# nurturenature/jepsen-tigerbeetle

Hardware: AMD Instinct MI355X
Metric: histories/sec, 10k-op/64-proc cas-register histories (time-to-verdict ms in extra) (higher is better)
Workload: dtype u64

## Files before the change

jepsen-tigerbeetle_amd/csrc/open_walk_impl.h:

```cpp
#pragma once
#include "wave_env.h"
#include "tbc_internal.h"

namespace tbc {
namespace walk {

constexpr uint32_t kCandCap = 136;
constexpr uint32_t kCandWords = 8;
constexpr uint32_t kAuxWords = 80;
constexpr uint32_t kKeyWords = 32, kKeyBits = 32 * kKeyWords;
static_assert(2 * kKeyWords <= kAuxWords && kKeyWords == 32, "the map and its prefix fit the scratch; two rows of 16 lanes scan it");
constexpr uint32_t kCursorWords = 64 + 32;
WV_HD constexpr uint32_t walk_lds_words() { return kCandCap * kCandWords + kAuxWords + kCursorWords; }
static_assert(4u * walk_lds_words() * sizeof(uint32_t) <= 20u * 1024u, "eight blocks of four wavefronts a CU");
constexpr uint32_t kTogWords = 64 * 4, kRankCntWords = 24;
constexpr uint32_t kSparseCand = kCandCap - (kTogWords + kRankCntWords) / kCandWords;
constexpr int kSparseSets = 2;
static_assert(kSparseCand <= 64u * kSparseSets, "two sets of 64 candidates");
static_assert((kTogWords + kRankCntWords) % kCandWords == 0u && (kSparseCand * kCandWords) % 4u == 0u && kSparseCand >= 96u, "the toggle words of a front are 16 bytes, aligned");
#ifndef TBC_WALK_BLOCKS
#define TBC_WALK_BLOCKS 8
#endif

constexpr uint32_t kCList = 1u;
constexpr uint32_t kCTwin = 2u;
constexpr uint32_t kCRow = 4u;
constexpr uint32_t kCLook = 8u;

WV_DEV void or_slot(uint32_t& lo, uint32_t& hi, bool cond, uint32_t slot) {
  if (slot < 32u) lo = wv::opaque(lo | (cond ? (1u << slot) : 0u));
  else hi = wv::opaque(hi | (cond ? (1u << (slot - 32u)) : 0u));
}
WV_DEV uint32_t effect_key(uint32_t f, int32_t a, int32_t b) {
  return (f & 3u) | (((uint32_t)a & 0x7FFFu) << 2) | ((f == TBC_F_CAS ? ((uint32_t)b & 0x7FFFu) : 0u) << 17);
}
static_assert(kMaxRuleValue < 0x7FFF && TBC_F_READ < 3 && TBC_F_WRITE < 3 && TBC_F_CAS < 3, "effect_key packs f and two rule values into a word, and no key has all bits set");
static_assert(kLookNone <= 0xFFu, "the produced value shares a word with the flags");

WV_DEV uint32_t rank_code(uint32_t slot, uint32_t f, int32_t a, uint32_t vpad) {
  return front_rank_code(slot, f == TBC_F_READ ? (rdm_index(a, vpad) & 0xFFu) : 0xFFu);
}

template <int Q>
WV_DEV void store_entries(const wv::u32x16& r, uint64_t* row, uint32_t n) {
  WV_UNROLL
  for (int v = 0; v < 8; v++) if ((uint32_t)(8 * Q + v) < n) row[8 * Q + v] = (uint64_t)r[2 * v] | ((uint64_t)r[2 * v + 1] << 32);
}

#ifndef TBC_WALK_RUN
#define TBC_WALK_RUN 8
#endif
constexpr uint32_t kWalkRun = TBC_WALK_RUN;
static_assert(kWalkRun >= 1u, "a run has a chunk");
constexpr uint32_t kStatWalkSearch = 40, kStatWalkCarried = 41, kStatWalkCursorMiss = 42;
constexpr uint32_t kStatWalkSparse = 43, kStatWalkDense = 44, kStatWalkEmitTrips = 45, kStatWalkTwinSteps = 46, kStatWalkRounds = 47, kStatWalkTwinFind = 48;
constexpr uint32_t kStatWalkCands = 49;
constexpr uint32_t kStatWalkFindWave = 52, kStatWalkChainWave = 53;
#if defined(TBC_EMU)
#define WV_STAT_WAVE_MAX(id, n) do { for (uint32_t k_ = 1u; wv::ballot((n) >= k_) != 0ull; k_++) if (lane == 0u) wv::stat((id), 1); } while (0)
#else
#define WV_STAT_WAVE_MAX(id, n) do { (void)(n); } while (0)
#endif

WV_DEV uint32_t xor_scan(uint32_t x, uint32_t lane) {
  x ^= wv::row_shr0<1>(x); x ^= wv::row_shr0<2>(x); x ^= wv::row_shr0<4>(x); x ^= wv::row_shr0<8>(x);
  const uint32_t t0 = wv::readlane(x, 15u), t1 = wv::readlane(x, 31u), t2 = wv::readlane(x, 47u);
  return x ^ (lane >= 16u ? t0 : 0u) ^ (lane >= 32u ? t1 : 0u) ^ (lane >= 48u ? t2 : 0u);
}
#ifndef TBC_WALK_OFF_AFTER
#define TBC_WALK_OFF_AFTER 1u
#endif
#if !defined(TBC_EMU) && (defined(TBC_WALK_TWIN_LE) || defined(TBC_WALK_NO_SELF_EXCLUSION) || (TBC_WALK_OFF_AFTER != 1u))
#error "the planted mutations of the front walk are for tests/emu (TBC_EMU) only"
#endif
WV_DEV void toggle_slot(uint32_t* tog, uint32_t F_lo, uint32_t inv, uint32_t ret, uint32_t slot) {
  if (ret < F_lo) return;
  const uint32_t on = inv > F_lo ? inv - F_lo : 0u, offi = ret + TBC_WALK_OFF_AFTER - F_lo, bit = 1u << (slot & 31u), w = slot >> 5;
  wv::lds_add32(&tog[on * 4u + w], bit);
  if (ret != kInf && offi < 64u) wv::lds_add32(&tog[offi * 4u + 2u + w], bit);
}
WV_DEV void zero_toggles(uint32_t* tog, uint32_t lane) {
  const uint32_t z = wv::opaque(0u);
  *reinterpret_cast<wv::u32x4*>(tog + lane * 4u) = wv::u32x4{z, z, z, z};
}
WV_DEV uint64_t open_bits(const uint32_t* tog, uint32_t lane, bool high) {
  wv::barrier();
  const wv::u32x4 t4 = *reinterpret_cast<const wv::u32x4*>(tog + lane * 4u);
  const uint32_t lo = xor_scan(t4.x ^ t4.z, lane), hi = high ? xor_scan(t4.y ^ t4.w, lane) : 0u;
  return (uint64_t)lo | ((uint64_t)hi << 32);
}
WV_DEV uint32_t next_pending(const bool (&pend)[kSparseSets], const uint32_t (&c_fl)[kSparseSets], uint32_t NC) {
  const uint64_t b0 = wv::ballot(pend[0]), b1 = NC > 64u ? wv::ballot(pend[1]) : 0ull;
  if ((b0 | b1) == 0ull) return 0u;
  return b0 ? wv::readlane(c_fl[0], (uint32_t)__builtin_ctzll(b0)) : wv::readlane(c_fl[1], (uint32_t)__builtin_ctzll(b1));
}
WV_DEV uint32_t key_bucket(uint32_t key) { return (key * 0x9E3779B1u) >> 26; }
#if defined(TBC_EMU)
inline bool& emu_force_dense() { static bool f = false; return f; }
#endif

#if defined(TBC_EMU)
WV_DEV uint32_t opaque_uniform(uint32_t v) { return v; }
#else
WV_DEV uint32_t opaque_uniform(uint32_t v) { asm volatile("" : "+s"(v)); return v; }
#endif

#if defined(TBC_EMU)
template <class T> using ro_t = const T;
#else
template <class T> using ro_t = const __attribute__((address_space(4))) T;
#endif
template <class T>
WV_DEV ro_t<T>* read_only(const T* p) { return (ro_t<T>*)(uintptr_t)p; }

WV_DEV uint32_t first_open(const Rec* rec, uint32_t l, uint32_t hi, uint32_t ret_from) {
  while (l < hi) {
    const uint32_t mid = (l + hi) >> 1;
    if (rec[mid].ret_rank >= ret_from) hi = mid; else l = mid + 1u;
  }
  return l;
}

struct Chunk {
  ro_t<PackOpenArgs>* A;
  ro_t<Hist>* H;
  ro_t<BeamHist>* B;
  uint32_t R, F_lo, F_hi, W;
  uint32_t ret_from;
  const Rec* rec; const uint32_t* seg; const uint32_t* off;
  OpRec* lst; uint64_t* twn;
  bool want_tw;
  uint32_t V, FW;
  bool compact;
  uint64_t* rdm; uint64_t* look;
  uint32_t *cand, *aux;
  uint16_t* perm;
  uint32_t* cur_end; uint16_t* cur_left;
  uint32_t *tog, *rcnt;
};

WV_DEV uint32_t fill_candidates(const Chunk& K, uint32_t lane, bool carried) {
  const Rec* rec = K.rec;
  const uint32_t* seg = K.seg;
  const uint32_t F_lo = K.F_lo, F_hi = K.F_hi, W = K.W, V = K.V, ret_from = K.ret_from;
  const uint32_t ret_from_next = K.look ? F_lo + 64u - (kLookahead - 1u) : F_lo + 64u;
  uint32_t lo = 0, k = 0;
  if (lane == 0u) wv::stat(carried ? kStatWalkCarried : kStatWalkSearch, 1);
  if (lane < W) {
    uint32_t i;
    if (carried) { i = K.cur_end[lane]; lo = i - K.cur_left[lane]; }
    else {
      lo = first_open(rec, seg[lane] + 1u, seg[lane + 1] - 1u, ret_from);
      i = lo;
    }
#if defined(TBC_EMU)
    if (carried && lo != first_open(rec, seg[lane] + 1u, seg[lane + 1] - 1u, ret_from)) wv::stat(kStatWalkCursorMiss, 1);
    if (i > seg[lane + 1] - 1u) wv::stat(kStatWalkCursorMiss, 1);
#endif
    const uint32_t last = read_only(seg)[W] - 1u;
    for (;;) {
      const uint32_t i1 = i + 1u < last ? i + 1u : last, i2 = i + 2u < last ? i + 2u : last, i3 = i + 3u < last ? i + 3u : last;
      const uint32_t v0 = rec[i].inv_rank, v1 = rec[i1].inv_rank, v2 = rec[i2].inv_rank, v3 = rec[i3].inv_rank;
      if (v0 >= F_hi) break;
      i++;
      if (v1 >= F_hi) break;
      i++;
      if (v2 >= F_hi) break;
      i++;
      if (v3 >= F_hi) break;
      i++;
    }
    k = i - lo;
  }
  uint32_t incl = k;
  for (uint32_t d = 1; d < 64u; d <<= 1) {
    K.aux[lane] = incl;
    wv::barrier();
    const uint32_t add = lane >= d ? K.aux[lane - d] : 0u;
    wv::barrier();
    incl += add;
  }
  const uint32_t base = incl - k;
  const uint32_t NC_all = wv::readlane(incl, 63u);
  uint32_t gone = 0;
  for (uint32_t j = 0; j < k; j++) {
    const Rec r = rec[lo + j];
    gone += r.ret_rank < ret_from_next ? 1u : 0u;
    if (base + j < kCandCap) {
      const bool live = (r.cls & 2u) != 0u, isread = (r.cls & 16u) != 0u, wc = (r.cls & 8u) != 0u;
      const bool in_chunk = r.ret_rank >= F_lo;
      const bool listed = live && in_chunk && !(K.A->branch_lists && isread);
      const uint32_t vi = rdm_index(r.a, V);
      uint32_t fl = (lane << 12) | (r.prod << 24);
      if (listed) fl |= kCList;
      if (listed && wc && K.want_tw) fl |= kCTwin;
      if (live && in_chunk && isread && K.rdm && V && (vi != 0u || r.a == TBC_NIL)) fl |= kCRow | (vi << 4);
      if (K.look && (r.cls & 6u) && r.prod != kLookNone) fl |= kCLook;
      uint32_t* e = K.cand + (base + j) * kCandWords;
      e[0] = r.inv_rank; e[1] = r.ret_rank; e[2] = r.opidx; e[3] = r.f | (lane << 8);
      e[4] = (uint32_t)r.a; e[5] = (uint32_t)r.b; e[6] = fl;
      e[7] = (live && wc && in_chunk) ? effect_key(r.f, r.a, r.b) : 0xFFFFFFFFu;
    }
  }
  K.cur_end[lane] = lo + k; K.cur_left[lane] = (uint16_t)(k - gone);
  wv::barrier();
  return NC_all;
}

WV_DEV void places_by_compare(uint32_t NC, const uint32_t (&my)[3], uint32_t (&place)[3]) {
  if (NC <= 64u) {
    for (uint32_t j = 0; j < NC; j++) place[0] += wv::readlane(my[0], j) < my[0] ? 1u : 0u;
  } else if (NC <= 128u) {
    for (uint32_t j = 0; j < 64u; j++) { const uint32_t kj = wv::readlane(my[0], j); place[0] += kj < my[0] ? 1u : 0u; place[1] += kj < my[1] ? 1u : 0u; }
    for (uint32_t j = 0; j < NC - 64u; j++) { const uint32_t kj = wv::readlane(my[1], j); place[0] += kj < my[0] ? 1u : 0u; place[1] += kj < my[1] ? 1u : 0u; }
  } else {
    WV_UNROLL
    for (int s2 = 0; s2 < 3; s2++) {
      const uint32_t cnt = s2 < 2 ? 64u : NC - 128u;
      for (uint32_t j = 0; j < cnt; j++) {
        const uint32_t kj = wv::readlane(my[s2], j);
        place[0] += kj < my[0] ? 1u : 0u; place[1] += kj < my[1] ? 1u : 0u; place[2] += kj < my[2] ? 1u : 0u;
      }
    }
  }
}
WV_DEV void places_by_counting(uint32_t* aux, uint32_t NC, uint32_t lane, const uint32_t (&d)[3], uint32_t (&place)[3]) {
  if (lane < kKeyWords) aux[lane] = 0u;
  wv::barrier();
  WV_UNROLL
  for (int s = 0; s < 3; s++) if (d[s] != kInf) wv::lds_add32(&aux[d[s] >> 5], 1u << (d[s] & 31u));
  wv::barrier();
  const uint32_t wc = lane < kKeyWords ? (uint32_t)__builtin_popcount(aux[lane]) : 0u;
  uint32_t y = wc;
  y += wv::row_shr0<1>(y); y += wv::row_shr0<2>(y); y += wv::row_shr0<4>(y); y += wv::row_shr0<8>(y);
  const uint32_t row0 = wv::readlane(y, 15u);
  y += lane >= 16u ? row0 : 0u;
  const uint32_t n_live = wv::readlane(y, kKeyWords - 1u);
  if (lane < kKeyWords) aux[kKeyWords + lane] = y - wc;
  const uint64_t below = (1ull << lane) - 1ull;
  uint32_t cr_before = n_live;
  WV_UNROLL
  for (int s = 0; s < 3; s++) {
    const uint32_t idx = lane + 64u * (uint32_t)s;
    const uint64_t cr = wv::ballot(idx < NC && d[s] == kInf);
    if (d[s] == kInf) place[s] = cr_before + (uint32_t)__builtin_popcountll(cr & below);
    cr_before += (uint32_t)__builtin_popcountll(cr);
  }
  wv::barrier();
  WV_UNROLL
  for (int s = 0; s < 3; s++)
    if (d[s] != kInf) place[s] = aux[kKeyWords + (d[s] >> 5)] + (uint32_t)__builtin_popcount(aux[d[s] >> 5] & ((1u << (d[s] & 31u)) - 1u));
  wv::barrier();
}
WV_DEV void list_places(const Chunk& K, uint32_t NC, uint32_t lane, uint32_t list_order, uint32_t (&place)[3]) {
  const uint32_t wr_last = list_order == 2u ? 0x40000000u : list_order >= 16u ? 2u * (list_order - 16u) + 1u : 0u;
  const uint32_t rk_mul = list_order >= 16u ? 2u : 1u;
  const uint32_t wr_ofs = list_order == 2u ? kKeyBits / 2u : wr_last, lim_other = list_order == 2u ? kKeyBits / 2u : kKeyBits;
  uint32_t my[3];
  uint32_t d[3];
  bool outside = false;
  WV_UNROLL
  for (int s = 0; s < 3; s++) {
    const uint32_t idx = lane + 64u * (uint32_t)s;
    const uint32_t* e = K.cand + (idx < NC ? idx : 0u) * kCandWords;
    const uint32_t rt = e[1];
    const bool wr = (e[3] & 0xFFu) == TBC_F_WRITE;
    my[s] = idx >= NC ? 0xFFFFFFFFu : rt == kInf ? (0xFFFFFF00u | idx) : rt * rk_mul + (wr ? wr_last : 0u);
    const bool live = idx < NC && rt != kInf;
    const uint32_t x = rt - K.ret_from;
    const bool inside = x < kKeyBits && x * rk_mul + (wr ? wr_ofs : 0u) < (wr ? kKeyBits : lim_other);
    d[s] = (live && inside) ? x * rk_mul + (wr ? wr_ofs : 0u) : kInf;
    outside = outside || (live && !inside);
    place[s] = 0u;
  }
  if (wr_ofs < kKeyBits && wv::ballot(outside) == 0ull) places_by_counting(K.aux, NC, lane, d, place);
  else places_by_compare(NC, my, place);
  WV_UNROLL
  for (int s = 0; s < 3; s++) {
    const uint32_t idx = lane + 64u * (uint32_t)s;
    if (idx < NC) K.perm[place[s]] = (uint16_t)idx;
  }
  wv::barrier();
}

WV_DEV void sparse_flags(const Chunk& K, uint32_t NC, uint32_t lane, const uint32_t (&place)[3], uint32_t (&c_fl)[kSparseSets]) {
  WV_UNROLL
  for (int s = 0; s < kSparseSets; s++) {
    const uint32_t idx = lane + 64u * (uint32_t)s;
    if (idx < NC) c_fl[s] = K.cand[idx * kCandWords + 6u] | ((place[s] & 63u) << 18) | ((place[s] >> 6) << 9);
  }
}
WV_DEV void dense_twin_keys(const Chunk& K, uint32_t NC, uint32_t lane, uint32_t (&c_key)[3], uint32_t (&c_ret)[3]) {
  WV_UNROLL
  for (int s = 0; s < 3; s++) {
    const uint32_t idx = lane + 64u * (uint32_t)s;
    const uint32_t* e = K.cand + (idx < NC ? idx : 0u) * kCandWords;
    c_key[s] = idx < NC ? e[7] : 0xFFFFFFFFu;
    c_ret[s] = e[1];
  }
}

WV_DEV void link_twins(const Chunk& K, uint32_t NC, uint32_t lane, uint32_t (&c_key)[3], uint32_t (&c_ret)[3]) {
  uint32_t* const cand = K.cand;
  uint32_t* const tog = K.tog;
  uint32_t prev[kSparseSets] = {0xFFu, 0xFFu}, prev_ret[kSparseSets] = {0u, 0u};
  WV_UNROLL
  for (int s = 0; s < kSparseSets; s++) {
    const uint32_t idx = lane + 64u * (uint32_t)s;
    if (idx < NC) { c_key[s] = cand[idx * kCandWords + 7u]; c_ret[s] = cand[idx * kCandWords + 1u]; }
  }
  WV_UNROLL
  for (int sp = 0; sp < kSparseSets; sp++) {
    if (64u * (uint32_t)sp >= NC) continue;
    { const uint32_t z = wv::opaque(0u); tog[lane * 2u] = z; tog[lane * 2u + 1u] = z; }
    wv::barrier();
    if (c_key[sp] != 0xFFFFFFFFu) wv::lds_add32(&tog[key_bucket(c_key[sp]) * 2u + (lane >> 5)], 1u << (lane & 31u));
    wv::barrier();
    WV_UNROLL
    for (int s = 0; s < kSparseSets; s++) {
      uint64_t mk = 0ull;
      if (c_key[s] != 0xFFFFFFFFu) {
        const uint32_t hb = key_bucket(c_key[s]);
        mk = (uint64_t)tog[hb * 2u] | ((uint64_t)tog[hb * 2u + 1u] << 32);
      }
      WV_STAT_WAVE_MAX(kStatWalkFindWave, (uint32_t)__builtin_popcountll(mk));
      while (mk) {
        const uint32_t u = 64u * (uint32_t)sp + (uint32_t)__builtin_ctzll(mk);
        mk &= mk - 1ull;
        const uint32_t* eu = cand + u * kCandWords;
        const uint32_t ru = eu[1];
        wv::stat(kStatWalkTwinFind, 1);
#if defined(TBC_WALK_TWIN_LE)
        if (eu[7] == c_key[s] && ru <= c_ret[s] && (prev[s] == 0xFFu || ru > prev_ret[s])) { prev[s] = u; prev_ret[s] = ru; }
#else
        if (eu[7] == c_key[s] && ru < c_ret[s] && (prev[s] == 0xFFu || ru > prev_ret[s])) { prev[s] = u; prev_ret[s] = ru; }
#endif
      }
    }
    wv::barrier();
  }
  WV_UNROLL
  for (int s = 0; s < kSparseSets; s++) if (lane + 64u * (uint32_t)s < NC) cand[(lane + 64u * (uint32_t)s) * kCandWords + 7u] = prev[s];
  wv::barrier();
}

struct Front {
  uint32_t F, Fc; bool active;
  uint32_t pos0, px, need, xprod, di, x, xf; int32_t xa;
};
WV_DEV Front front_of(const Chunk& K, uint32_t lane) {
  const auto& A = *K.A;
  const auto* H = K.H;
  Front f;
  f.F = K.F_lo + lane;
  f.active = f.F < K.F_hi;
  f.Fc = f.active ? f.F : K.F_hi - 1u;
  f.pos0 = K.off[f.Fc];
  f.px = A.ret_slot[H->ret_off + f.Fc];
  f.need = kLookNone; f.xprod = kLookNone; f.di = 0; f.x = 0; f.xf = kFNone; f.xa = 0;
  if (K.look || K.compact) {
    f.x = A.ret_op[H->ret_off + f.Fc];
    f.xf = A.f[H->op_off + f.x];
    f.xa = A.a[H->op_off + f.x];
  }
  if (K.look) {
    const int32_t xb = A.b[H->op_off + f.x];
    const uint32_t xinv = A.scratch[H->frame_off + f.x];
    f.need = look_need(f.xf, f.xa); f.xprod = look_prod(f.xf, f.xa, xb);
    f.di = f.F - xinv < 255u ? f.F - xinv : 255u;
  }
  return f;
}
WV_DEV void store_look(const Chunk& K, const Front& f, uint64_t pm, uint32_t dmin) {
  if (f.active && K.look) {
    pm &= ~(1ull << (f.px & 63u));
    K.look[(uint64_t)f.F * 2u] = look_word0(f.px, f.need, f.xprod, f.di, dmin);
    K.look[(uint64_t)f.F * 2u + 1u] = pm;
  }
}

WV_DEV void sparse_read_rows(const Chunk& K, uint32_t NC, uint32_t lane, const Front& f, const uint32_t (&c_fl)[kSparseSets]) {
  uint64_t* const row = K.rdm ? K.rdm + (uint64_t)f.F * K.FW : nullptr;
  const uint32_t n_row = K.compact ? 6u : K.V;
  uint32_t made = 0u;
  bool pend[kSparseSets];
  WV_UNROLL
  for (int s = 0; s < kSparseSets; s++) pend[s] = (c_fl[s] & kCRow) != 0u;
  for (uint32_t fl; (fl = next_pending(pend, c_fl, NC)) != 0u;) {
    const uint32_t v = (fl >> 4) & 31u;
    if (lane == 0u) wv::stat(kStatWalkRounds, 1);
    zero_toggles(K.tog, lane);
    wv::barrier();
    WV_UNROLL
    for (int s = 0; s < kSparseSets; s++)
      if (pend[s] && ((c_fl[s] >> 4) & 31u) == v) { const uint32_t* e = K.cand + (lane + 64u * (uint32_t)s) * kCandWords; toggle_slot(K.tog, K.F_lo, e[0], e[1], (c_fl[s] >> 12) & 63u); pend[s] = false; }
    const uint64_t open = open_bits(K.tog, lane, K.W > 32u);
    if (f.active && v < n_row) row[v] = open;
    made |= 1u << v;
    wv::barrier();
  }
  if (K.rdm)
    for (uint32_t v = 0; v < n_row; v++) if (!((made >> v) & 1u) && f.active) row[v] = 0ull;
}
WV_DEV void sparse_producers(const Chunk& K, uint32_t NC, uint32_t lane, const Front& f, const uint32_t (&c_fl)[kSparseSets]) {
  static_assert(kLookahead == 8u, "a front's window of invocation ranks is eight bytes");
  uint32_t* const rcnt = K.rcnt;
  uint64_t pm = 0ull;
  uint32_t dmin = 255u;
  bool pend[kSparseSets];
  WV_UNROLL
  for (int s = 0; s < kSparseSets; s++) pend[s] = (c_fl[s] & kCLook) != 0u;
  for (uint32_t fl; (fl = next_pending(pend, c_fl, NC)) != 0u;) {
    const uint32_t v = fl >> 24;
    const bool mine = f.active && f.need == v;
    if (wv::ballot(mine) == 0ull) {
      WV_UNROLL
      for (int s = 0; s < kSparseSets; s++) if ((c_fl[s] >> 24) == v) pend[s] = false;
      continue;
    }
    if (lane == 0u) wv::stat(kStatWalkRounds, 1);
    zero_toggles(K.tog, lane);
    if (lane < kRankCntWords) rcnt[lane] = 0u;
    wv::barrier();
    WV_UNROLL
    for (int s = 0; s < kSparseSets; s++)
      if (pend[s] && (c_fl[s] >> 24) == v) {
        const uint32_t* e = K.cand + (lane + 64u * (uint32_t)s) * kCandWords;
        const uint32_t inv = e[0];
        toggle_slot(K.tog, K.F_lo, inv, e[1], (c_fl[s] >> 12) & 63u);
        if (inv + (kLookahead - 1u) >= K.F_lo) {
          const uint32_t ri = inv + (kLookahead - 1u) - K.F_lo;
          wv::lds_add32(&rcnt[ri >> 2], 1u << (8u * (ri & 3u)));
        }
        pend[s] = false;
      }
    const uint64_t open = open_bits(K.tog, lane, K.W > 32u);
    if (mine) {
      pm = open;
      const uint32_t wb = lane >> 2, sh = 8u * (lane & 3u);
      const uint64_t lo64 = (uint64_t)rcnt[wb] | ((uint64_t)rcnt[wb + 1u] << 32);
      uint64_t xb = sh ? ((lo64 >> sh) | ((uint64_t)rcnt[wb + 2u] << (64u - sh))) : lo64;
#if !defined(TBC_WALK_NO_SELF_EXCLUSION)
      if (f.xprod == f.need && f.di < kLookahead) xb -= 1ull << (8u * (kLookahead - 1u - f.di));
#endif
      dmin = xb ? (uint32_t)__builtin_clzll(xb) >> 3 : 255u;
    }
    wv::barrier();
  }
  store_look(K, f, pm, dmin);
}
WV_DEV uint32_t sparse_lists(const Chunk& K, uint32_t NC, uint32_t lane, const Front& f, const uint32_t (&c_fl)[kSparseSets], bool by_ret, uint32_t pos) {
  const uint32_t* const cand = K.cand;
  const uint32_t F = f.F;
  WV_UNROLL
  for (int g = 0; g < kSparseSets; g++) {
    if (64u * (uint32_t)g >= NC) continue;
    zero_toggles(K.tog, lane);
    wv::barrier();
    WV_UNROLL
    for (int s = 0; s < kSparseSets; s++)
      if ((c_fl[s] & kCList) && ((c_fl[s] >> 9) & 3u) == (uint32_t)g) { const uint32_t* e = cand + (lane + 64u * (uint32_t)s) * kCandWords; toggle_slot(K.tog, K.F_lo, e[0], e[1], (c_fl[s] >> 18) & 63u); }
    const uint64_t open = open_bits(K.tog, lane, true);
    uint64_t cur = f.active ? open : 0ull;
    wv::barrier();
    WV_NOUNROLL
    while (wv::ballot(cur != 0ull) != 0ull) {
      if (lane == 0u) wv::stat(kStatWalkEmitTrips, 1);
      uint32_t chain_steps = 0u;
      if (cur != 0ull) {
        const uint32_t p = 64u * (uint32_t)g + (uint32_t)__builtin_ctzll(cur);
        cur &= cur - 1ull;
        const uint32_t* e = cand + (by_ret ? (uint32_t)K.perm[p] : p) * kCandWords;
        OpRec o; o.op = e[2]; o.f_slot = e[3] | (e[1] == F ? kAtFront : 0u); o.a = (int32_t)e[4]; o.b = (int32_t)e[5];
        K.lst[pos] = o;
        if (K.twn) {
          uint64_t tw = 0ull;
          for (uint32_t u = e[7] & 0xFFu; u != 0xFFu;) {
            const uint32_t* eu = cand + u * kCandWords;
            wv::stat(kStatWalkTwinSteps, 1);
            chain_steps++;
            if (eu[1] < F) break;
            if (eu[0] <= F) tw |= 1ull << ((eu[3] >> 8) & 63u);
#if defined(TBC_WALK_TWIN_LE)
            if ((eu[7] & 0xFFu) == u) break;
#endif
            u = eu[7] & 0xFFu;
          }
          K.twn[pos] = tw;
        }
        pos++;
      }
      WV_STAT_WAVE_MAX(kStatWalkChainWave, chain_steps);
    }
  }
  return pos;
}

template <int VCAP>
WV_DEV uint32_t dense_loop(const Chunk& K, uint32_t NC, uint32_t lane, const Front& f, const uint32_t (&c_key)[3], const uint32_t (&c_ret)[3], bool by_ret, uint32_t pos) {
  const uint32_t* const cand = K.cand;
  const uint32_t F = f.F;
  const bool active = f.active;
  wv::u32x16 r0, r1, r2, r3;
  WV_UNROLL
  for (int i = 0; i < 16; i++) { r0[i] = 0u; r1[i] = 0u; r2[i] = 0u; r3[i] = 0u; }
  uint32_t pm_lo = 0u, pm_hi = 0u, dmin = 255u;
  WV_NOUNROLL
  for (uint32_t t = 0; t < NC; t++) {
    const uint32_t* e = cand + (by_ret ? (uint32_t)K.perm[t] : t) * kCandWords;
    const uint32_t inv = e[0], ret = e[1];
    const uint32_t fl = wv::readfirstlane(e[6]);
    const uint32_t slot = (fl >> 12) & 63u;
    const bool member = active && inv <= F && F <= ret;
    if (fl & kCList) {
      uint32_t tw_lo = 0u, tw_hi = 0u;
      if (fl & kCTwin) {
        const uint32_t key_t = e[7];
        uint64_t s0 = wv::ballot(c_key[0] == key_t && c_ret[0] < ret && c_ret[0] >= inv);
        uint64_t s1 = 0ull, s2 = 0ull;
        if (NC > 64u) s1 = wv::ballot(c_key[1] == key_t && c_ret[1] < ret && c_ret[1] >= inv);
        if (NC > 128u) s2 = wv::ballot(c_key[2] == key_t && c_ret[2] < ret && c_ret[2] >= inv);
        while (s0 | s1 | s2) {
          uint32_t u;
          if (s0) { u = (uint32_t)__builtin_ctzll(s0); s0 &= s0 - 1ull; }
          else if (s1) { u = 64u + (uint32_t)__builtin_ctzll(s1); s1 &= s1 - 1ull; }
          else { u = 128u + (uint32_t)__builtin_ctzll(s2); s2 &= s2 - 1ull; }
          const uint32_t* eu = cand + u * kCandWords;
          const bool mu = eu[0] <= F && F <= eu[1];
          or_slot(tw_lo, tw_hi, mu, (wv::readfirstlane(eu[6]) >> 12) & 63u);
        }
      }
      if (member) {
        OpRec o; o.op = e[2]; o.f_slot = e[3] | (ret == F ? kAtFront : 0u); o.a = (int32_t)e[4]; o.b = (int32_t)e[5];
        K.lst[pos] = o;
        if (K.twn) K.twn[pos] = (uint64_t)tw_lo | ((uint64_t)tw_hi << 32);
        pos++;
      }
    }
    if (fl & kCRow)
    {
      const uint32_t w = ((fl >> 4) & 31u) * 2u + (slot >> 5), bit = member ? (1u << (slot & 31u)) : 0u;
      if constexpr (VCAP <= 8) r0[w & 15u] |= bit;
      else {
        const uint32_t q = w >> 4;
        if (q == 0u) r0[w & 15u] |= bit; else if (q == 1u) r1[w & 15u] |= bit; else if (q == 2u) r2[w & 15u] |= bit; else r3[w & 15u] |= bit;
      }
    }
    if (fl & kCLook) {
      const bool hit = (fl >> 24) == f.need;
      or_slot(pm_lo, pm_hi, member && hit, slot);
      const uint32_t dist = F - inv;
      if (hit && dist < kLookahead && e[2] != f.x) dmin = dist < dmin ? dist : dmin;
    }
  }
  if (active && K.rdm) {
    uint64_t* row = K.rdm + (uint64_t)F * K.FW;
    const uint32_t n_row = K.compact ? 6u : K.V;
    store_entries<0>(r0, row, n_row);
    if constexpr (VCAP > 8) { store_entries<1>(r1, row, n_row); store_entries<2>(r2, row, n_row); store_entries<3>(r3, row, n_row); }
  }
  store_look(K, f, (uint64_t)pm_lo | ((uint64_t)pm_hi << 32), dmin);
  return pos;
}

WV_DEV void compact_tail(const Chunk& K, uint32_t lane, const Front& f, bool by_ret, uint32_t nl) {
  const auto& A = *K.A;
  const auto* H = K.H;
  uint32_t* const aux = K.aux;
  if (by_ret) wv::barrier();
  aux[lane] = f.active ? rank_code(f.px, f.xf, f.xa, K.V) : (7u << 6);
  if (lane < kFrontCompactRanks - 1u) {
    const uint32_t G = K.F_lo + 64u + lane;
    uint32_t code = 7u << 6;
    if (G < K.R) {
      const uint32_t gx = A.ret_op[H->ret_off + G];
      code = rank_code(A.ret_slot[H->ret_off + G], A.f[H->op_off + gx], A.a[H->op_off + gx], K.V);
    }
    aux[64u + lane] = code;
  }
  wv::barrier();
  uint64_t w7 = 0ull;
  WV_UNROLL
  for (uint32_t l = kFrontCompactRanks; l-- > 0u;) w7 |= (uint64_t)aux[lane + l] << (9u * l);
  const uint64_t w6 = front_word6(f.pos0, nl, A.ncr[K.B->off_off + f.Fc]);
  if (f.active && K.rdm) {
    uint64_t* row = K.rdm + (uint64_t)f.F * K.FW;
    row[6] = w6; row[7] = w7;
  }
}

template <int VCAP>
WV_DEV bool walk_chunk(const PackOpenArgs& A_, uint32_t h, uint32_t c, uint32_t* lds, uint32_t lane, bool carried) {
  const auto& A = *wv::cold(A_);
  const auto* H = read_only(&A.hist[h]);
  const auto* B = read_only(&A.bh[h]);
  const uint32_t R = H->n_ret;
  const uint32_t F_lo = c * 64u;
  if (H->status != 0 || B->status != 0 || F_lo >= R) return false;
  Chunk K;
  K.A = &A; K.H = H; K.B = B;
  K.R = R; K.F_lo = F_lo; K.F_hi = F_lo + 64u < R ? F_lo + 64u : R;
  K.W = H->n_slots;
  K.rec = A.rec + H->rec_off;
  K.seg = A.seg + H->seg_off;
  K.off = A.off + B->off_off;
  K.lst = A.lst + B->lst_off;
  K.twn = A.twn ? A.twn + B->lst_off : nullptr;
  K.want_tw = K.twn != nullptr;
  K.V = A.vpad;
  K.FW = A.front_words ? A.front_words : K.V;
  K.compact = A.front_compact != 0u;
  K.rdm = (A.rdm && (K.V || K.compact)) ? A.rdm + H->op_off * K.FW : nullptr;
  K.look = A.look ? A.look + look_off(H->op_off, h, 1u) : nullptr;
  K.ret_from = K.look ? (F_lo >= kLookahead - 1u ? F_lo - (kLookahead - 1u) : 0u) : F_lo;
  K.cand = lds;
  K.aux = lds + kCandCap * kCandWords;
  K.perm = reinterpret_cast<uint16_t*>(K.aux);
  K.cur_end = K.aux + kAuxWords;
  K.cur_left = reinterpret_cast<uint16_t*>(K.cur_end + 64);
  K.tog = K.cand + kSparseCand * kCandWords;
  K.rcnt = K.tog + kTogWords;

  const uint32_t NC_all = fill_candidates(K, lane, carried);
  const uint32_t NC = NC_all < kCandCap ? NC_all : kCandCap;
  const uint32_t list_order = A.order_of ? A.order_of[h] : A.list_order;
  const bool by_ret = list_order != 0u;
  uint32_t place[3] = {lane, lane + 64u, lane + 128u};
  if (by_ret) list_places(K, NC, lane, list_order, place);

  bool sparse = VCAP <= 8 && NC_all <= kSparseCand;
#if defined(TBC_EMU)
  if (emu_force_dense()) sparse = false;
#endif
  uint32_t c_fl[kSparseSets] = {0u, 0u};
  uint32_t c_key[3] = {0xFFFFFFFFu, 0xFFFFFFFFu, 0xFFFFFFFFu}, c_ret[3] = {0u, 0u, 0u};
  if (sparse) sparse_flags(K, NC, lane, place, c_fl);
  else if (K.want_tw) dense_twin_keys(K, NC, lane, c_key, c_ret);
  if constexpr (VCAP <= 8) if (sparse && K.want_tw) link_twins(K, NC, lane, c_key, c_ret);
  if (lane == 0u) wv::stat(sparse ? kStatWalkSparse : kStatWalkDense, 1);
  if (lane == 0u) wv::stat(kStatWalkCands + (NC_all > 64u ? 1u : 0u) + (NC_all > kSparseCand ? 1u : 0u), 1);

  const Front f = front_of(K, lane);
  uint32_t pos = f.pos0;
  bool dense = true;
  if constexpr (VCAP <= 8) if (sparse) {
    dense = false;
    sparse_read_rows(K, NC, lane, f, c_fl);
    sparse_producers(K, NC, lane, f, c_fl);
    pos = sparse_lists(K, NC, lane, f, c_fl, by_ret, pos);
  }
  if (dense) pos = dense_loop<VCAP>(K, NC, lane, f, c_key, c_ret, by_ret, pos);
  if (K.compact) compact_tail(K, lane, f, by_ret, pos - f.pos0);
  return F_lo + 64u < R;
}

template <int VCAP>
WV_DEV void walk_wave(const PackOpenArgs& A, uint32_t wid, uint32_t* lds, uint32_t lane) {
  const uint32_t cph = A.chunks_per_hist;
  const uint32_t hr = wid / cph, c = wid - hr * cph, h = A.h0 + hr;
  if (h >= A.n_hist) return;
  (void)walk_chunk<VCAP>(A, h, c, lds, lane, false);
}

WV_HD constexpr uint32_t walk_runs_per_hist(uint32_t chunks_per_hist, uint32_t run = kWalkRun) { return (chunks_per_hist + run - 1u) / run; }

template <int VCAP, uint32_t RUN = kWalkRun>
WV_DEV void walk_run(const PackOpenArgs& A, uint32_t run_id, uint32_t* lds, uint32_t lane) {
  const uint32_t rph = walk_runs_per_hist(A.chunks_per_hist, RUN);
  const uint32_t hr = run_id / rph, c0 = (run_id - hr * rph) * RUN, h = A.h0 + hr;
  if (h >= A.n_hist) return;
  WV_NOUNROLL
  for (uint32_t j = 0; j < RUN; j++) {
    if (!walk_chunk<VCAP>(A, opaque_uniform(h), c0 + j, lds, wv::opaque(lane), j != 0u)) break;
    wv::barrier();
  }
}

}
}
```

Before: 410,200.

## Redistribute sparse list emission across lanes by global entry rank

The sparse emission loop no longer has each lane (front) walk its own open candidates serially. It computes a wave-wide prefix sum of per-front counts, then assigns every output entry to a lane in batches of 64. Each lane finds its front through an LDS mark array and a max-scan, then locates the k-th set bit of that front's open mask. The aim is to remove divergence where one busy front serialises the wave, and to make the lst/twn writes contiguous across lanes. In exchange it adds LDS round-trips, barriers and scans per batch, and it assumes the fronts' output positions are contiguous.

```diff
diff --git a/jepsen-tigerbeetle_amd/csrc/open_walk_impl.h b/jepsen-tigerbeetle_amd/csrc/open_walk_impl.h
--- a/jepsen-tigerbeetle_amd/csrc/open_walk_impl.h
+++ b/jepsen-tigerbeetle_amd/csrc/open_walk_impl.h
@@ -56,10 +56,18 @@
 constexpr uint32_t kStatWalkSparse = 43, kStatWalkDense = 44, kStatWalkEmitTrips = 45, kStatWalkTwinSteps = 46, kStatWalkRounds = 47, kStatWalkTwinFind = 48;
 constexpr uint32_t kStatWalkCands = 49;
 constexpr uint32_t kStatWalkFindWave = 52, kStatWalkChainWave = 53;
+constexpr uint32_t kStatWalkEntries = 54, kStatWalkNotContiguous = 55, kStatWalkBadPlace = 56, kStatWalkSecondSet = 57;
+constexpr uint32_t kStatWalkLstLines = 58;
 #if defined(TBC_EMU)
 #define WV_STAT_WAVE_MAX(id, n) do { for (uint32_t k_ = 1u; wv::ballot((n) >= k_) != 0ull; k_++) if (lane == 0u) wv::stat((id), 1); } while (0)
+#define WV_STAT_WAVE_LINES(id, on, at) do { uint32_t n_ = 0u; uint64_t seen_[64]; \
+    for (uint32_t j_ = 0u; j_ < 64u; j_++) { const uint64_t l_ = wv::readlane64((on) ? ((uint64_t)(at) >> 7) + 1ull : 0ull, j_); bool new_ = l_ != 0ull; \
+      for (uint32_t i_ = 0u; i_ < n_; i_++) new_ = new_ && seen_[i_] != l_; \
+      if (new_) seen_[n_++] = l_; } \
+    if (lane == 0u) wv::stat((id), n_); } while (0)
 #else
 #define WV_STAT_WAVE_MAX(id, n) do { (void)(n); } while (0)
+#define WV_STAT_WAVE_LINES(id, on, at) do { } while (0)
 #endif
 
 WV_DEV uint32_t xor_scan(uint32_t x, uint32_t lane) {
@@ -449,9 +457,31 @@
   }
   store_look(K, f, pm, dmin);
 }
-WV_DEV uint32_t sparse_lists(const Chunk& K, uint32_t NC, uint32_t lane, const Front& f, const uint32_t (&c_fl)[kSparseSets], bool by_ret, uint32_t pos) {
+WV_DEV uint32_t kth_set_bit(const wv::u32x4& t, uint32_t k) {
+  const uint32_t c0 = (uint32_t)__builtin_popcount(t.x), c1 = c0 + (uint32_t)__builtin_popcount(t.y), c2 = c1 + (uint32_t)__builtin_popcount(t.z);
+  uint32_t w = t.x, p = 0u;
+  if (k >= c2) { w = t.w; p = 96u; k -= c2; } else if (k >= c1) { w = t.z; p = 64u; k -= c1; } else if (k >= c0) { w = t.y; p = 32u; k -= c0; }
+  WV_UNROLL
+  for (uint32_t s = 16u; s != 0u; s >>= 1) {
+    const uint32_t c = (uint32_t)__builtin_popcount(w & ((1u << s) - 1u));
+    if (k >= c) { k -= c; w >>= s; p += s; }
+  }
+  return p;
+}
+WV_DEV uint32_t max_scan(uint32_t x, uint32_t lane) {
+  const auto mx = [](uint32_t a, uint32_t b) { return a > b ? a : b; };
+  x = mx(x, wv::row_shr0<1>(x)); x = mx(x, wv::row_shr0<2>(x)); x = mx(x, wv::row_shr0<4>(x)); x = mx(x, wv::row_shr0<8>(x));
+  const uint32_t t0 = wv::readlane(x, 15u), t1 = wv::readlane(x, 31u), t2 = wv::readlane(x, 47u);
+  return mx(mx(x, lane >= 16u ? t0 : 0u), mx(lane >= 32u ? t1 : 0u, lane >= 48u ? t2 : 0u));
+}
+#if !defined(TBC_EMU) && (defined(TBC_WALK_RANK_OFF_BY_ONE) || defined(TBC_WALK_FRONT_LE))
+#error "the planted mutations of the front walk are for tests/emu (TBC_EMU) only"
+#endif
+WV_DEV uint32_t sparse_lists(const Chunk& K, uint32_t NC, uint32_t lane, const Front& f, const uint32_t (&c_fl)[kSparseSets], bool by_ret) {
+  static_assert(kSparseSets == 2 && kTogWords == 64u * 4u && kRankCntWords >= 16u, "a front's two sets are its four toggle words; 64 mark bytes");
   const uint32_t* const cand = K.cand;
-  const uint32_t F = f.F;
+  uint32_t* const mark = K.rcnt;
+  uint64_t open[kSparseSets] = {0ull, 0ull};
   WV_UNROLL
   for (int g = 0; g < kSparseSets; g++) {
     if (64u * (uint32_t)g >= NC) continue;
@@ -460,40 +490,87 @@
     WV_UNROLL
     for (int s = 0; s < kSparseSets; s++)
       if ((c_fl[s] & kCList) && ((c_fl[s] >> 9) & 3u) == (uint32_t)g) { const uint32_t* e = cand + (lane + 64u * (uint32_t)s) * kCandWords; toggle_slot(K.tog, K.F_lo, e[0], e[1], (c_fl[s] >> 18) & 63u); }
-    const uint64_t open = open_bits(K.tog, lane, true);
-    uint64_t cur = f.active ? open : 0ull;
-    wv::barrier();
-    WV_NOUNROLL
-    while (wv::ballot(cur != 0ull) != 0ull) {
-      if (lane == 0u) wv::stat(kStatWalkEmitTrips, 1);
-      uint32_t chain_steps = 0u;
-      if (cur != 0ull) {
-        const uint32_t p = 64u * (uint32_t)g + (uint32_t)__builtin_ctzll(cur);
-        cur &= cur - 1ull;
-        const uint32_t* e = cand + (by_ret ? (uint32_t)K.perm[p] : p) * kCandWords;
-        OpRec o; o.op = e[2]; o.f_slot = e[3] | (e[1] == F ? kAtFront : 0u); o.a = (int32_t)e[4]; o.b = (int32_t)e[5];
-        K.lst[pos] = o;
-        if (K.twn) {
-          uint64_t tw = 0ull;
-          for (uint32_t u = e[7] & 0xFFu; u != 0xFFu;) {
-            const uint32_t* eu = cand + u * kCandWords;
-            wv::stat(kStatWalkTwinSteps, 1);
-            chain_steps++;
-            if (eu[1] < F) break;
-            if (eu[0] <= F) tw |= 1ull << ((eu[3] >> 8) & 63u);
+    const uint64_t o = open_bits(K.tog, lane, true);
+    open[g] = f.active ? o : 0ull;
+    wv::barrier();
+  }
+  *reinterpret_cast<wv::u32x4*>(K.tog + lane * 4u) = wv::u32x4{(uint32_t)open[0], (uint32_t)(open[0] >> 32), (uint32_t)open[1], (uint32_t)(open[1] >> 32)};
+  const uint32_t n = (uint32_t)__builtin_popcountll(open[0]) + (uint32_t)__builtin_popcountll(open[1]);
+  uint32_t incl = n;
+  incl += wv::row_shr0<1>(incl); incl += wv::row_shr0<2>(incl); incl += wv::row_shr0<4>(incl); incl += wv::row_shr0<8>(incl);
+  {
+    const uint32_t t0 = wv::readlane(incl, 15u), t1 = t0 + wv::readlane(incl, 31u), t2 = t1 + wv::readlane(incl, 47u);
+    incl += lane >= 48u ? t2 : lane >= 32u ? t1 : lane >= 16u ? t0 : 0u;
+  }
+  const uint32_t start = incl - n, total = wv::readlane(incl, 63u);
+  const uint32_t base = wv::readlane(f.pos0, 0u);
+#if defined(TBC_EMU)
+  if (f.active && f.pos0 != base + start) wv::stat(kStatWalkNotContiguous, 1);
+  if (lane == 0u) wv::stat(kStatWalkEntries, total);
+#endif
+  uint32_t carry_front = 0u, carry_start = 0u;
+  WV_NOUNROLL
+  for (uint32_t e0 = 0u; e0 < total; e0 += 64u) {
+    if (lane == 0u) wv::stat(kStatWalkEmitTrips, 1);
+    if (lane < 16u) mark[lane] = wv::opaque(0u);
+    wv::barrier();
+#if defined(TBC_WALK_FRONT_LE)
+    if (n != 0u && !(start <= e0) && start - e0 < 64u)
+#else
+    if (n != 0u && !(start < e0) && start - e0 < 64u)
+#endif
+      wv::lds_add32(&mark[(start - e0) >> 2], (0x40u | lane) << (8u * ((start - e0) & 3u)));
+    wv::barrier();
+    const uint32_t mb = (mark[lane >> 2] >> (8u * (lane & 3u))) & 0xFFu;
+    const uint32_t mv = max_scan(mb ? (0x1000u | ((mb & 63u) << 6) | lane) : 0u, lane);
+    const uint32_t fr = mv ? (mv >> 6) & 63u : carry_front;
+#if defined(TBC_WALK_RANK_OFF_BY_ONE)
+    const uint32_t k = (mv ? lane - (mv & 63u) : e0 + lane - carry_start) + 1u;
+#else
+    const uint32_t k = mv ? lane - (mv & 63u) : e0 + lane - carry_start;
+#endif
+    {
+      const uint32_t last = wv::readlane(mv, 63u);
+      if (last != 0u) { carry_front = (last >> 6) & 63u; carry_start = e0 + (last & 63u); }
+    }
+    uint32_t chain_steps = 0u;
+    if (e0 + lane < total) {
+      const uint32_t F = K.F_lo + fr;
+      const wv::u32x4 sets = *reinterpret_cast<const wv::u32x4*>(K.tog + fr * 4u);
+      const uint32_t p = kth_set_bit(sets, k);
+      uint32_t ci = by_ret ? (uint32_t)K.perm[p] : p;
+#if defined(TBC_EMU)
+      if (p >= 64u) wv::stat(kStatWalkSecondSet, 1);
+      if (ci >= NC || k >= (uint32_t)__builtin_popcount(sets.x) + (uint32_t)__builtin_popcount(sets.y) + (uint32_t)__builtin_popcount(sets.z) + (uint32_t)__builtin_popcount(sets.w)) {
+        wv::stat(kStatWalkBadPlace, 1);
+        ci = 0u;
+      }
+#endif
+      const uint32_t* e = cand + ci * kCandWords;
+      const uint64_t at = (uint64_t)base + e0 + lane;
+      OpRec o; o.op = e[2]; o.f_slot = e[3] | (e[1] == F ? kAtFront : 0u); o.a = (int32_t)e[4]; o.b = (int32_t)e[5];
+      K.lst[at] = o;
+      if (K.twn) {
+        uint64_t tw = 0ull;
+        for (uint32_t u = e[7] & 0xFFu; u != 0xFFu;) {
+          const uint32_t* eu = cand + u * kCandWords;
+          wv::stat(kStatWalkTwinSteps, 1);
+          chain_steps++;
+          if (eu[1] < F) break;
+          if (eu[0] <= F) tw |= 1ull << ((eu[3] >> 8) & 63u);
 #if defined(TBC_WALK_TWIN_LE)
-            if ((eu[7] & 0xFFu) == u) break;
-#endif
-            u = eu[7] & 0xFFu;
-          }
-          K.twn[pos] = tw;
+          if ((eu[7] & 0xFFu) == u) break;
+#endif
+          u = eu[7] & 0xFFu;
         }
-        pos++;
-      }
-      WV_STAT_WAVE_MAX(kStatWalkChainWave, chain_steps);
-    }
-  }
-  return pos;
+        K.twn[at] = tw;
+      }
+    }
+    WV_STAT_WAVE_MAX(kStatWalkChainWave, chain_steps);
+    WV_STAT_WAVE_LINES(kStatWalkLstLines, e0 + lane < total, (K.B->lst_off + base + e0 + lane) * sizeof(OpRec));
+    wv::barrier();
+  }
+  return f.pos0 + n;
 }
 
 template <int VCAP>
@@ -647,7 +724,7 @@
     dense = false;
     sparse_read_rows(K, NC, lane, f, c_fl);
     sparse_producers(K, NC, lane, f, c_fl);
-    pos = sparse_lists(K, NC, lane, f, c_fl, by_ret, pos);
+    pos = sparse_lists(K, NC, lane, f, c_fl, by_ret);
   }
   if (dense) pos = dense_loop<VCAP>(K, NC, lane, f, c_key, c_ret, by_ret, pos);
   if (K.compact) compact_tail(K, lane, f, by_ret, pos - f.pos0);
```

Result: faster. 427,100 (median of 6 runs) (+4.1%).
